# rasmusab/bayes.js

Hardware: AMD Instinct MI355X
Metric: posterior draws/sec (= param-updates/sec) (higher is better)
Workload: dtype f64

## Files before the change

bayes.js_amd/amwg_ctypes.py:

```python
import ctypes as C
import os

import numpy as np

HERE = os.path.dirname(os.path.abspath(__file__))
LIB_PATH = os.environ.get("AMWG_LIB") or os.path.join(HERE, "csrc", "libamwg.so")
MODEL_ID = {"normal": 1, "beta_bern": 2, "hier_normal": 3, "pois_glm": 4}


class ParamDesc(C.Structure):
    _fields_ = [("type", C.c_int32), ("len", C.c_int32), ("top", C.c_int32), ("multidim", C.c_int32),
                ("lower", C.c_double), ("upper", C.c_double)]


class CompOpt(C.Structure):
    _fields_ = [("prop_log_scale", C.c_double), ("max_adaptation", C.c_double), ("initial_adaptation", C.c_double),
                ("target_accept_rate", C.c_double), ("batch_size", C.c_double), ("is_adapting", C.c_int32)]


class ModelDesc(C.Structure):
    _fields_ = [("model", C.c_int32), ("n_obs", C.c_int32), ("x", C.POINTER(C.c_double)), ("y", C.POINTER(C.c_double)),
                ("g", C.POINTER(C.c_int32)), ("G", C.c_int32), ("K", C.c_int32), ("hyper", C.c_double * 8)]


DEFAULT_HYPER = {"normal": [0, 100, 0, 100], "beta_bern": [2, 2], "hier_normal": [0, 100, 0, 100, 10], "pois_glm": [0, 10]}


class Options(C.Structure):
    _fields_ = [("chains", C.c_int64), ("seed", C.c_uint64), ("chain_offset", C.c_uint64), ("device", C.c_int32),
                ("lanes_per_chain", C.c_int32), ("block_threads", C.c_int32), ("steps_per_launch", C.c_int32),
                ("exact_division", C.c_int32), ("group_local", C.c_int32), ("full_evaluation", C.c_int32), ("test_bound_shift", C.c_int32), ("sufficient_statistics", C.c_int32)]


class UserModel(C.Structure):
    _fields_ = [("source", C.c_char_p), ("n_arrays", C.c_int32), ("arrays", C.POINTER(C.POINTER(C.c_double))),
                ("array_len", C.POINTER(C.c_int64)), ("array_type", C.POINTER(C.c_int32)), ("n_derived", C.c_int32), ("lds_bytes", C.c_int32), ("lds_bytes_one_lane", C.c_int32),
                ("parallel", C.c_int32), ("max_threads", C.c_int32), ("work_per_eval", C.c_double), ("work_one_lane", C.c_double),
                ("rows_n_obs", C.c_int32), ("rows_groups", C.c_int32), ("rows_sweep", C.c_int32)]


EXPORTS = ["amwg_kernel_name", "amwg_summation_order", "amwg_group_gather_draws", "amwg_group_comm_info", "amwg_comm_unique_id", "amwg_comm_create", "amwg_comm_info", "amwg_comm_gather_draws", "amwg_comm_moments", "amwg_comm_destroy", "amwg_code_cache_stats", "amwg_tuning", "amwg_group_moments", "amwg_group_diagnostics", "amwg_group_quantiles", "amwg_last_sample_quantiles", "amwg_fp64_peak", "amwg_set_state", "amwg_last_sample_diagnostics", "amwg_create_user", "amwg_compile_user", "amwg_num_recorded", "amwg_create", "amwg_burn", "amwg_burn_async", "amwg_sample", "amwg_sample_async", "amwg_fetch_draws", "amwg_fetch_draws_slices", "amwg_sample_device", "amwg_set_adapting", "amwg_get_state", "amwg_info", "amwg_chain_diag", "amwg_last_sample_moments", "amwg_sync", "amwg_num_components", "amwg_num_chains", "amwg_launch_info", "amwg_destroy", "amwg_last_error", "amwg_version", "amwg_exp", "amwg_log", "amwg_uniform"]
SELFTEST_EXPORTS = ["amwg_prefault_selftest", "amwg_math1", "amwg_math2", "amwg_hypot3", "amwg_log1p", "amwg_expm1", "amwg_two_valued_sum_check", "amwg_pow", "amwg_ld_host", "amwg_ld_device", "amwg_device_eval"]

_lib = None


def lib():
    global _lib
    if _lib is None:
        if not os.path.exists(LIB_PATH):
            raise RuntimeError("libamwg.so is missing: run `python -c 'import __graft_entry__ as g; g.build()'`")
        L = C.CDLL(LIB_PATH)
        vp, i32, i64, u64, dbl = C.c_void_p, C.c_int32, C.c_int64, C.c_uint64, C.c_double
        pd, pi32, pi64, pu64 = C.POINTER(dbl), C.POINTER(i32), C.POINTER(i64), C.POINTER(u64)
        L.amwg_create.argtypes = [C.POINTER(ModelDesc), C.POINTER(ParamDesc), i32, pd, C.POINTER(CompOpt),
                                  C.POINTER(Options), C.POINTER(vp)]
        L.amwg_burn.argtypes = [vp, i64]
        L.amwg_burn_async.argtypes = [vp, i64]
        L.amwg_sample_async.argtypes = [vp, i64, i64]
        L.amwg_fetch_draws.argtypes = [vp, pd, C.c_size_t]
        L.amwg_fetch_draws_slices.argtypes = [vp, C.c_int32, C.POINTER(C.c_int32), C.POINTER(C.c_int32), C.POINTER(C.POINTER(C.c_double)), C.POINTER(C.c_size_t)]
        L.amwg_sample.argtypes = [vp, i64, i64, pd, C.c_size_t]
        L.amwg_sample_device.argtypes = [vp, i64, i64, vp, C.c_size_t]
        L.amwg_set_adapting.argtypes = [vp, i32]
        L.amwg_get_state.argtypes = [vp, pd, C.c_size_t]
        L.amwg_info.argtypes = [vp, pd, pi32, pi32, pi32, pi64, pi64]
        L.amwg_chain_diag.argtypes = [vp, pu64, pd, pi32]
        L.amwg_last_sample_moments.argtypes = [vp, pd, pd]
        L.amwg_sync.argtypes = [vp]
        L.amwg_num_components.argtypes = [vp]
        L.amwg_num_chains.argtypes = [vp]
        L.amwg_num_chains.restype = i64
        L.amwg_launch_info.argtypes = [vp, pi32, pi32, pi32, pi32, pi32, pd]
        L.amwg_kernel_name.argtypes = [vp]
        L.amwg_summation_order.argtypes = [vp]
        L.amwg_kernel_name.restype = C.c_char_p
        L.amwg_destroy.argtypes = [vp]
        L.amwg_last_error.restype = C.c_char_p
        L.amwg_version.restype = C.c_char_p
        L.amwg_exp.restype = dbl
        L.amwg_exp.argtypes = [dbl]
        L.amwg_log.restype = dbl
        L.amwg_log.argtypes = [dbl]
        L.amwg_uniform.restype = dbl
        L.amwg_uniform.argtypes = [u64, u64, u64]
        L.amwg_compile_user.argtypes = [C.c_char_p, i32, i32, C.c_char_p, C.POINTER(C.c_size_t)]
        L.amwg_code_cache_stats.argtypes = [pi64, pi64, C.c_char_p, C.c_size_t]
        L.amwg_create_user.argtypes = [C.POINTER(UserModel), C.POINTER(ParamDesc), i32, pd, C.POINTER(CompOpt),
                                       C.POINTER(Options), C.POINTER(vp)]
        L.amwg_num_recorded.argtypes = [vp]
        L.amwg_set_state.argtypes = [vp, pd, C.c_size_t]
        L.amwg_fp64_peak.argtypes = [i32, pd]
        L.amwg_last_sample_quantiles.argtypes = [vp, pd, i32, pd]
        L.amwg_last_sample_diagnostics.argtypes = [vp, pd, pd]
        pvp = C.POINTER(vp)
        L.amwg_group_moments.argtypes = [pvp, i32, pd, pd]
        L.amwg_group_diagnostics.argtypes = [pvp, i32, pd, pd]
        L.amwg_group_quantiles.argtypes = [pvp, i32, pd, i32, pd]
        L.amwg_group_gather_draws.argtypes = [pvp, i32, i32, vp, pd, C.c_size_t, pi64]
        L.amwg_group_comm_info.argtypes = [pvp, i32, pi32, pi32, i32]
        L.amwg_comm_unique_id.argtypes = [C.c_char_p, C.c_size_t]
        L.amwg_comm_create.argtypes = [C.c_char_p, C.c_size_t, i32, i32, i32, pvp]
        L.amwg_comm_info.argtypes = [vp, pi32, pi32, pi32]
        L.amwg_comm_gather_draws.argtypes = [vp, vp, i32, vp, C.c_size_t, pi64]
        L.amwg_comm_moments.argtypes = [vp, vp, pd, pd]
        L.amwg_comm_destroy.argtypes = [vp]
        _lib = L
    return _lib


_selftest = None


def selftest_lib():
    global _selftest
    if _selftest is None:
        path = os.path.join(os.path.dirname(LIB_PATH), "libamwg_selftest.so")
        if not os.path.exists(path):
            raise RuntimeError("libamwg_selftest.so is missing: run `python -c 'import __graft_entry__ as g; g.build()'`")
        L = C.CDLL(path)
        i32, i64, dbl = C.c_int32, C.c_int64, C.c_double
        pd = C.POINTER(dbl)
        L.amwg_last_error.restype = C.c_char_p
        L.amwg_device_eval.argtypes = [i32, i32, i64, pd, pd, pd, pd]
        L.amwg_two_valued_sum_check.argtypes = [i32, pd, i32, i64, pd, pd, pd, pd, pd]
        L.amwg_pow.restype = dbl
        L.amwg_pow.argtypes = [dbl, dbl]
        L.amwg_math1.restype = dbl
        L.amwg_math1.argtypes = [i32, dbl]
        L.amwg_math2.restype = dbl
        L.amwg_math2.argtypes = [i32, dbl, dbl]
        L.amwg_hypot3.restype = dbl
        L.amwg_hypot3.argtypes = [dbl, dbl, dbl]
        for f in ("amwg_log1p", "amwg_expm1"):
            getattr(L, f).restype = dbl
            getattr(L, f).argtypes = [dbl]
        L.amwg_ld_host.restype = dbl
        L.amwg_ld_host.argtypes = [i32, dbl, dbl, dbl, dbl]
        L.amwg_ld_device.argtypes = [i32, i64, pd, pd]
        L.amwg_prefault_selftest.argtypes = [C.c_void_p, C.c_size_t, i32, i32]
        _selftest = L
    return _selftest


class AmwgError(RuntimeError):
    pass


def _check(rc):
    if rc != 0:
        raise AmwgError("amwg error %d: %s" % (rc, lib().amwg_last_error().decode()))


def _dp(a):
    return a.ctypes.data_as(C.POINTER(C.c_double))


class Sampler:

    def __init__(self, spec, chains, seed, chain_offset=0, device=0, lanes_per_chain=0, block_threads=0,
                 steps_per_launch=0, exact_division=0, group_local=0, full_evaluation=0, test_bound_shift=0, sufficient_statistics=0):
        L = lib()
        keep = []
        user = spec.get("user")
        if user is None:
            d = spec["data"]
            md = ModelDesc()
            md.model = MODEL_ID[spec["model"]]
            md.n_obs = spec["n_obs"]
            x = np.ascontiguousarray(d["x"], dtype=np.float64)
            keep.append(x)
            md.x = _dp(x)
            if "y" in d:
                y = np.ascontiguousarray(d["y"], dtype=np.float64)
                keep.append(y)
                md.y = _dp(y)
            if "g" in d:
                g = np.ascontiguousarray(d["g"], dtype=np.int32)
                keep.append(g)
                md.g = g.ctypes.data_as(C.POINTER(C.c_int32))
            md.G = int(spec.get("G", 0))
            md.K = int(spec.get("K", 0))
            for i, v in enumerate(spec.get("hyper") or DEFAULT_HYPER[spec["model"]]):
                md.hyper[i] = float(v)
        else:
            um = UserModel()
            src = user["source"].encode() if isinstance(user["source"], str) else user["source"]
            keep.append(src)
            um.source = src
            arrs = [np.ascontiguousarray(a, dtype=np.float64) for a in user["arrays"]]
            keep.append(arrs)
            um.n_arrays = len(arrs)
            ptrs = (C.POINTER(C.c_double) * max(1, len(arrs)))(*[_dp(a) for a in arrs])
            lens = (C.c_int64 * max(1, len(arrs)))(*[a.size for a in arrs])
            types = (C.c_int32 * max(1, len(arrs)))(*[int(t) for t in user.get("array_types", [0] * len(arrs))])
            keep += [ptrs, lens, types]
            um.arrays, um.array_len, um.array_type = ptrs, lens, types
            um.n_derived, um.lds_bytes = int(user.get("n_derived", 0)), int(user.get("lds_bytes", 0))
            um.lds_bytes_one_lane = int(user.get("lds_bytes_one_lane", 0))
            um.parallel, um.max_threads = int(user.get("parallel", 0)), int(user.get("max_threads", 0))
            um.work_per_eval = float(user.get("work_per_eval", 0.0))
            um.work_one_lane = float(user.get("work_one_lane", 0.0))
            um.rows_n_obs, um.rows_groups, um.rows_sweep = int(user.get("rows_n_obs", 0)), int(user.get("rows_groups", 0)), int(user.get("rows_sweep", 0))
        n = len(spec["params"])
        pa = (ParamDesc * n)()
        TYPE = {"real": 0, "int": 1, "binary": 2}
        for i, p in enumerate(spec["params"]):
            pa[i].type = TYPE[p["type"]]
# ... 242 lines not shown
```

bayes.js_amd/csrc/amwg_models.h:

```cpp
#pragma once
#include "amwg_div.h"
#include "amwg_ld.h"
#include "amwg_pass.h"
#include "amwg_twoval.h"
#include "amwg_types.h"
#include "amwg_window.h"

namespace amwg {

__device__ __forceinline__ double norm_const_sd(double v, double m, double c_sd, double den, double y_hi, double y_lo, int den_ok) {
  const double t = v - m;
  const double tt = t * t;
  const double q = (den_ok && wide_range(tt)) ? div_by_invariant(tt, den, Reciprocal{y_hi, y_lo}) : tt / den;
  return c_sd - q;
}

struct NormCache {
  double sd, c, den;
  Reciprocal y;
  bool den_ok;
};
__device__ __forceinline__ NormCache norm_cache_init() { return NormCache{__builtin_nan(""), 0.0, 0.0, Reciprocal{0.0, 0.0}, false}; }
AMWG_HD NormCache norm_cache_make(double sd, double neg_half_log_2pi) {
  NormCache k;
  k.sd = sd;
  k.c = norm_c(neg_half_log_2pi, sd);
  k.den = norm_den(sd);
  k.y = make_reciprocal(k.den);
  k.den_ok = mid_range(k.den);
  return k;
}
struct NormCacheA { double c, den; };
AMWG_HD_OUTLINE NormCacheA norm_cache_cold_a(double sd, double neg_half_log_2pi) { return NormCacheA{norm_c(neg_half_log_2pi, sd), norm_den(sd)}; }
AMWG_HD_OUTLINE Reciprocal norm_cache_cold_b(double den) { return make_reciprocal(den); }
template <bool COLD = false>
__device__ __forceinline__ void norm_cache_update(NormCache &k, double sd, double neg_half_log_2pi) {
  if (sd != k.sd) {
    if constexpr (COLD) {
      const NormCacheA a = norm_cache_cold_a(sd, neg_half_log_2pi);
      k.sd = sd; k.c = a.c; k.den = a.den;
      k.y = norm_cache_cold_b(a.den);
      k.den_ok = mid_range(a.den);
    } else {
      k = norm_cache_make(sd, neg_half_log_2pi);
    }
  }
}



struct NormalModel {
  static constexpr bool kSplitPrior = false;
  static constexpr bool kUser = false, kHasFast = true, kOneLanePass = false;
  static constexpr int kDerived = 0;
  static constexpr bool kHasBinary = false;
  static constexpr int kMaxThreads = 1024;
  static constexpr int kUnroll = 8;
  struct Pass { double mu, c, den; Reciprocal y; bool fast; const double *x; };
  static constexpr size_t kOneLaneTileLimit = 96 * 1024;
  __host__ __device__ static size_t one_lane_tile_bytes(int n_obs) { return (size_t)n_obs * 8 <= kOneLaneTileLimit ? (size_t)n_obs * 8 : 0; }
  __host__ __device__ static size_t lds_bytes(int n_obs, int, int lanes) { return lanes == 1 ? 0 : (size_t)n_obs * 8; }
  static constexpr bool kDynamicLds = true;
  __host__ __device__ static size_t lds_bytes_of(const DataRef &d, int lanes, int) { return lanes == 1 ? (d.pad > 0 ? one_lane_tile_bytes(d.n_obs) : 0) : (size_t)d.n_obs * 8; }
  __device__ static void stage(unsigned char *smem, const DataRef &d, int tid, int nt, int lanes) {
    if (lanes == 1 && lds_bytes_of(d, 1, nt) == 0) return;
    double *dst = reinterpret_cast<double *>(smem);
    for (int i = tid; i < d.n_obs; i += nt) dst[i] = d.x[i];
  }
  template <class C>
  __device__ __forceinline__ static double prior(const StateView &, const ModelConsts &mc, const DataRef &, C &kc) {
    double lp = 0;
    lp += norm_const_sd(kc.mu, mc.m0, mc.c0, mc.den0, mc.y0_hi, mc.y0_lo, mc.den0_ok);
    const double sigma = kc.sigma;
    lp += (sigma < mc.ua || sigma > mc.ub) ? -kInf : mc.lunif;
    return lp;
  }
  static constexpr bool kTracksState = true;
  struct Cache { NormCache n; double mu, sigma; bool loaded; };
  __device__ __forceinline__ static Cache cache_init() { return Cache{norm_cache_init(), 0.0, 0.0, false}; }
  __device__ __forceinline__ static void on_set(Cache &k, int comp, double v, int, const DataRef &) { k.mu = comp == 0 ? v : k.mu; k.sigma = comp == 0 ? k.sigma : v; }
  static constexpr bool kMirrorCheck = true;
  template <int GL>
  __device__ __forceinline__ static bool mirror_ok(const Cache &k, const StateView &S, const DataRef &, int) {
    return !k.loaded || (f64_bits(k.mu) == f64_bits(S(0)) && f64_bits(k.sigma) == f64_bits(S(1)));
  }
  template <int GL>
  __device__ __forceinline__ static void load(Cache &k, const StateView &S, const ModelConsts &, const DataRef &, const unsigned char *, int) {
    if (!k.loaded) { k.mu = S(0); k.sigma = S(1); k.loaded = true; }
  }
  template <int GL>
  __device__ __forceinline__ static Pass begin(const StateView &, const ModelConsts &mc, const DataRef &d,
                                               const unsigned char *smem, Cache &kc) {
    Pass ps;
    NormCache &k = kc.n;
    ps.mu = kc.mu;
    norm_cache_update(k, kc.sigma, mc.neg_half_log_2pi);
    ps.c = k.c;
    ps.den = k.den;
    ps.y = k.y;
    ps.fast = !mc.exact_division && mc.data_mid_range && k.den_ok &&
              (ps.mu == 0 || mid_range(__builtin_fabs(ps.mu)));
    ps.x = GL == 1 ? d.x : reinterpret_cast<const double *>(smem);
    return ps;
  }
  template <bool FAST>
  __device__ __forceinline__ static double term(const Pass &ps, int i) {
    const double t = ps.x[i] - ps.mu;
    const double tt = t * t;
    return ps.c - (FAST ? div_by_invariant(tt, ps.den, ps.y) : tt / ps.den);
  }
  template <int G>
  __device__ inline __attribute__((noinline)) static double pass_slow_impl(const double *x, double mu, double c, double den, int n_obs, int sub, double acc) {
    for (int i = sub; i < n_obs; i += G) { const double t = x[i] - mu; acc += c - (t * t) / den; }
    return acc;
  }
  template <int G>
  __device__ __forceinline__ static double pass_slow(const Pass &ps, int n_obs, int sub, double acc) { return pass_slow_impl<G>(ps.x, ps.mu, ps.c, ps.den, n_obs, sub, acc); }
  static constexpr bool kStagedFast = true;
  template <int G, int U = 8>
  __device__ __forceinline__ static double pass_fast(const Pass &ps, int n_obs, int sub, double acc) {
    if constexpr (G == 1) return norm_pass_uniform<8>(ps.x, ps.mu, ps.c, ps.den, ps.y, n_obs, acc);
    else return norm_pass_staged<G, U, false>(ps.x, nullptr, StateView{nullptr}, ps.mu, ps.c, ps.den, ps.y, n_obs, sub, acc);
  }
  static constexpr bool kCertified = true;
  static constexpr int kCertifiedLanes = 1;
  struct Approx { double value, eps; };
  template <int G, int BT>
  __device__ __forceinline__ static Approx log_post_approx(Cache &kc, const StateView &S, const ModelConsts &mc, const DataRef &d, const unsigned char *smem, int sub) {
    static_assert(G == 1, "the certified pass of the Normal family is the one-lane one");
    load<G>(kc, S, mc, d, smem, sub);
    norm_cache_update(kc.n, kc.sigma, mc.neg_half_log_2pi);
    const double P = prior(S, mc, d, kc);
    double S2;
    if (mc.sufficient) {
      const double dm = (mc.suff_xbar_hi - kc.mu) + mc.suff_xbar_lo;
      S2 = __builtin_fma((double)d.n_obs, dm * dm, mc.suff_ss);
    } else
    if constexpr (BT <= 512) S2 = norm_sq_pass_wave<(BT <= 256 ? kWaveBlock : 8)>(lds_bytes_of(d, 1, 0) ? reinterpret_cast<const double *>(smem) : d.x, kc.mu, d.n_obs, wave_scratch_of(d));
    else S2 = norm_sq_pass_uniform<8>(d.x, kc.mu, d.n_obs);
    const double n = (double)d.n_obs;
    const double Q = S2 * kc.n.y.hi, nc = n * kc.n.c;
    const double mag = __builtin_fabs(P) + __builtin_fabs(nc) + 2.0 * Q;
    return Approx{(P + nc) - Q, (2.0 * n + 64.0) * 0x1p-53 * mag * 1.25};
  }
};

struct BetaBernModel {
  static constexpr bool kSplitPrior = false;
  static constexpr bool kUser = false, kHasFast = false, kOneLanePass = true;
  static constexpr int kDerived = 0;
  static constexpr bool kHasBinary = false;
  static constexpr int kMaxThreads = 1024;
  static constexpr int kUnroll = 8;
  struct Pass { double l1, l0; const uint8_t *x; const uint32_t *bits; bool has_invalid, fast_forward; BitData B; };
  __host__ __device__ static size_t words(int n_obs) { return (size_t)n_obs / 32 + 2; }
  static constexpr size_t kFfLdsLimit = 120 * 1024;
  __host__ __device__ static size_t lds_bytes(int n_obs, int, int lanes) {
    if (lanes == 1) { const size_t b = 6 * words(n_obs) * 4; return b <= kFfLdsLimit ? ((b + 15) & ~(size_t)15) : 0; }
    return ((size_t)n_obs + 15) & ~(size_t)15;
  }
  __device__ static void stage(unsigned char *smem, const DataRef &d, int tid, int nt, int lanes) {
    if (lanes == 1) {
      if (lds_bytes(d.n_obs, 0, 1) == 0) return;
      uint32_t *dst = reinterpret_cast<uint32_t *>(smem);
      const uint32_t *src = static_cast<const uint32_t *>(d.arr[0]);
      for (int k = tid; k < (int)(6 * words(d.n_obs)); k += nt) dst[k] = src[k];
      return;
    }
    for (int i = tid; i < d.n_obs; i += nt) smem[i] = d.xb[i];
  }
  template <class C>
  __device__ __forceinline__ static double prior(const StateView &S, const ModelConsts &mc, const DataRef &, C &) {
    const double th = S(0);
    double lp = 0;
    if (th > 1 || th < 0) lp += -kInf;
    else if (mc.ba == 1 && mc.bb == 1) lp += 0.0;
    else lp += (mc.ba - 1) * log_v8(th) + (mc.bb - 1) * log_v8(1 - th) - mc.lbeta_ab;
    return lp;
  }
  struct Cache {};
  __device__ __forceinline__ static Cache cache_init() { return Cache{}; }
  template <int GL>
  __device__ __forceinline__ static Pass begin(const StateView &S, const ModelConsts &mc, const DataRef &d,
                                               const unsigned char *smem, Cache &) {
    Pass ps;
    const double th = S(0);
    ps.l1 = log_v8(th);
    ps.l0 = log_v8(1 - th);
    ps.x = smem;
    ps.bits = d.xw;
    ps.has_invalid = mc.has_invalid != 0;
    ps.fast_forward = !mc.exact_division;
    {
      const size_t W = words(d.n_obs);
      const uint32_t *base = lds_bytes(d.n_obs, 0, 1) ? reinterpret_cast<const uint32_t *>(smem) : static_cast<const uint32_t *>(d.arr[0]);
      ps.B.w = base; ps.B.pre = base + W; ps.B.om1 = base + 2 * W; ps.B.po1 = base + 3 * W; ps.B.om0 = base + 4 * W; ps.B.po0 = base + 5 * W;
      ps.B.n = d.n_obs;
    }
    return ps;
  }
  template <bool FAST>
  __device__ __forceinline__ static double term(const Pass &ps, int i) { return ps.x[i] ? ps.l1 : ps.l0; }

#define AMWG_A0 "v_add_f64 %[acc], %[acc], %[l0]\n"
#define AMWG_A1 "v_add_f64 %[acc], %[acc], %[l1]\n"
#define AMWG_N0 AMWG_A0 AMWG_A0 AMWG_A0 AMWG_A0
#define AMWG_N1 AMWG_A1 AMWG_A0 AMWG_A0 AMWG_A0
#define AMWG_N2 AMWG_A0 AMWG_A1 AMWG_A0 AMWG_A0
#define AMWG_N3 AMWG_A1 AMWG_A1 AMWG_A0 AMWG_A0
#define AMWG_N4 AMWG_A0 AMWG_A0 AMWG_A1 AMWG_A0
#define AMWG_N5 AMWG_A1 AMWG_A0 AMWG_A1 AMWG_A0
#define AMWG_N6 AMWG_A0 AMWG_A1 AMWG_A1 AMWG_A0
#define AMWG_N7 AMWG_A1 AMWG_A1 AMWG_A1 AMWG_A0
#define AMWG_N8 AMWG_A0 AMWG_A0 AMWG_A0 AMWG_A1
#define AMWG_N9 AMWG_A1 AMWG_A0 AMWG_A0 AMWG_A1
#define AMWG_N10 AMWG_A0 AMWG_A1 AMWG_A0 AMWG_A1
#define AMWG_N11 AMWG_A1 AMWG_A1 AMWG_A0 AMWG_A1
#define AMWG_N12 AMWG_A0 AMWG_A0 AMWG_A1 AMWG_A1
#define AMWG_N13 AMWG_A1 AMWG_A0 AMWG_A1 AMWG_A1
#define AMWG_N14 AMWG_A0 AMWG_A1 AMWG_A1 AMWG_A1
#define AMWG_N15 AMWG_A1 AMWG_A1 AMWG_A1 AMWG_A1
// ... 805 lines not shown
```

bayes.js_amd/csrc/amwg_pass.h:

```cpp
#pragma once
#include "amwg_div.h"
#include "amwg_types.h"

namespace amwg {

#if defined(__HIP_DEVICE_COMPILE__)
#define AMWG_STAGE_FENCE() __builtin_amdgcn_sched_barrier(0)
#else
#define AMWG_STAGE_FENCE() ((void)0)
#endif

template <int U>
struct NormBlock { double v[U]; };

#if defined(__HIP_DEVICE_COMPILE__)
#define AMWG_WAIT_LDS_LE(n) __builtin_amdgcn_s_waitcnt(0xC07F | ((n) << 8))
#else
#define AMWG_WAIT_LDS_LE(n) ((void)0)
#endif

template <int U, bool ADD_PREV>
AMWG_HD void norm_block_stages(NormBlock<U> &b, const double (&m)[U], NormBlock<U> &q, const NormBlock<U> &prev, double &acc,
                                                  double c, double den, Reciprocal y) {
  int a = 0;
// ... 184 lines not shown
    compute(sb, StagedFirst{});
    int ch = 1;
    for (; ch + 1 < n_chunks; ch += 2) {
      AMWG_WAIT_LDS_LE(0); AMWG_STAGE_FENCE();
      load_chunk(ch + 1, sb);
      AMWG_STAGE_FENCE();
      compute(sa, StagedLater{});
      AMWG_WAIT_LDS_LE(0); AMWG_STAGE_FENCE();
      load_chunk(ch + 2, sa);
      AMWG_STAGE_FENCE();
      compute(sb, StagedLater{});
    }
    if (ch < n_chunks) {
      AMWG_WAIT_LDS_LE(0); AMWG_STAGE_FENCE();
      compute(sa, StagedLater{});
    }
#pragma unroll
    for (int u = 0; u < U; ++u) acc = acc + qb.v[u];
    k = n_chunks * CH;
  }
  for (; k < n_obs; ++k) {
    const double t = x_global[k] - mean;
    acc += c - div_by_invariant(t * t, den, y);
  }
  return acc;
}

template <int U>
AMWG_HD double norm_sq_pass_uniform(const double *x_global, double mean, int n_obs) {
  constexpr int CH = 2 * U;
  double acc[U];
#pragma unroll
  for (int u = 0; u < U; ++u) acc[u] = 0.0;
  const int n_chunks = n_obs / CH;
  int k = 0;
  if (n_chunks > 0) {
    amwg_uniform_f64_ptr px = (amwg_uniform_f64_ptr)(uintptr_t)x_global;
    NormBlock<CH> sa, sb;
    auto load_chunk = [&](int ch, NormBlock<CH> &dst) {
      ch = ch < n_chunks ? ch : n_chunks - 1;
#pragma unroll
      for (int u = 0; u < CH; ++u) dst.v[u] = px[ch * CH + u];
    };
    auto compute = [&](const NormBlock<CH> &src) {
#pragma unroll
      for (int u = 0; u < U; ++u) { const double t = src.v[u] - mean; acc[u] = __builtin_fma(t, t, acc[u]); }
      AMWG_STAGE_FENCE();
#pragma unroll
      for (int u = 0; u < U; ++u) { const double t = src.v[U + u] - mean; acc[u] = __builtin_fma(t, t, acc[u]); }
      AMWG_STAGE_FENCE();
    };
    load_chunk(0, sb);
    AMWG_WAIT_LDS_LE(0); AMWG_STAGE_FENCE();
    load_chunk(1, sa);
    AMWG_STAGE_FENCE();
    compute(sb);
    int ch = 1;
    for (; ch + 1 < n_chunks; ch += 2) {
      AMWG_WAIT_LDS_LE(0); AMWG_STAGE_FENCE();
      load_chunk(ch + 1, sb);
      AMWG_STAGE_FENCE();
      compute(sa);
      AMWG_WAIT_LDS_LE(0); AMWG_STAGE_FENCE();
      load_chunk(ch + 2, sa);
      AMWG_STAGE_FENCE();
      compute(sb);
    }
    if (ch < n_chunks) {
      AMWG_WAIT_LDS_LE(0); AMWG_STAGE_FENCE();
      compute(sa);
    }
    k = n_chunks * CH;
  }
  for (; k < n_obs; ++k) {
    const double t = x_global[k] - mean;
    acc[0] = __builtin_fma(t, t, acc[0]);
  }
  double s = 0.0;
#pragma unroll
  for (int u = 0; u < U; ++u) s += acc[u];
  return s;
}

#if defined(__HIPCC__) || defined(__HIPCC_RTC__)
#ifndef AMWG_WAVE_BLOCK
#define AMWG_WAVE_BLOCK 16
#endif
constexpr int kWaveBlock = AMWG_WAVE_BLOCK;
template <int N> struct PassBlock { static constexpr int value = N; };
typedef int amwg_v16i __attribute__((ext_vector_type(16)));
__device__ __forceinline__ double *wave_scratch_of(const DataRef &d) {
#if defined(__HIP_DEVICE_COMPILE__)
  if (!d.wave_scratch) return nullptr;
  const uint32_t wave = (uint32_t)__builtin_amdgcn_readfirstlane((int)(blockIdx.x * (blockDim.x >> 6) + (threadIdx.x >> 6)));
  return d.wave_scratch + (size_t)wave * 64;
#else
  (void)d; return nullptr;
#endif
}
template <int B>
__device__ __forceinline__ double norm_sq_pass_wave(const double *x, double mu, int n_obs, double *scr = nullptr) {
#if defined(__HIP_DEVICE_COMPILE__)
  const int lane = (int)(threadIdx.x & 63u);
  double a[64];
#pragma unroll
  for (int c = 0; c < 64; ++c) a[c] = 0.0;
  const int mu_lo = (int)(uint32_t)f64_bits(mu), mu_hi = (int)(uint32_t)(f64_bits(mu) >> 32);
  auto mean_of = [&](int c) { return bits_f64(((uint64_t)(uint32_t)__builtin_amdgcn_readlane(mu_hi, c) << 32) | (uint64_t)(uint32_t)__builtin_amdgcn_readlane(mu_lo, c)); };
  bool smem_done = false;
#if !defined(AMWG_X_NO_SMEM_MEANS)
  if (scr != nullptr) {
    scr[lane] = mu;
    asm volatile("s_waitcnt vmcnt(0)\n\ts_dcache_inv\n\ts_waitcnt lgkmcnt(0)" ::: "memory");
    auto fetch = [&](int g) { amwg_v16i r; asm volatile("s_load_dwordx16 %0, %1, %2" : "=&s"(r) : "s"(scr), "s"(g * 8)); return r; };
    auto landed = [&](amwg_v16i &r) { asm volatile("s_waitcnt lgkmcnt(0)" : "+s"(r)); };
    auto mean_in = [&](const amwg_v16i &r, int j) { return bits_f64(((uint64_t)(uint32_t)r[2 * j + 1] << 32) | (uint64_t)(uint32_t)r[2 * j]); };
    auto block_s = [&](auto tag, int at) {
      constexpr int BB = decltype(tag)::value;
      double xv[BB];
      amwg_v16i cur = fetch(0);
#pragma unroll
      for (int b = 0; b < BB; ++b) xv[b] = x[at + b * 64 + lane];
#pragma unroll
      for (int g = 0; g < 64; g += 8) {
        landed(cur);
        amwg_v16i nxt = cur;
        if (g + 8 < 64) nxt = fetch(g + 8);
#pragma unroll
        for (int b = 0; b < BB; ++b) {
#pragma unroll
          for (int j = 0; j < 8; ++j) { const double t = xv[b] - mean_in(cur, j); a[g + j] = __builtin_fma(t, t, a[g + j]); }
        }
        cur = nxt;
      }
    };
    int base = 0;
    for (; base + 64 * B <= n_obs; base += 64 * B) block_s(PassBlock<B>{}, base);
    if constexpr (B >= 32) { if (base + 64 * 16 <= n_obs) { block_s(PassBlock<16>{}, base); base += 64 * 16; } }
    if constexpr (B >= 16) { if (base + 64 * 8 <= n_obs) { block_s(PassBlock<8>{}, base); base += 64 * 8; } }
    if constexpr (B >= 8) { if (base + 64 * 4 <= n_obs) { block_s(PassBlock<4>{}, base); base += 64 * 4; } }
    if constexpr (B >= 4) { if (base + 64 * 2 <= n_obs) { block_s(PassBlock<2>{}, base); base += 64 * 2; } }
    for (; base + 64 <= n_obs; base += 64) block_s(PassBlock<1>{}, base);
    if (base < n_obs) {
      const int i = base + lane;
      const bool has = i < n_obs;
      const double xv = x[has ? i : base];
      amwg_v16i cur = fetch(0);
#pragma unroll
      for (int g = 0; g < 64; g += 8) {
        landed(cur);
        amwg_v16i nxt = cur;
        if (g + 8 < 64) nxt = fetch(g + 8);
#pragma unroll
        for (int j = 0; j < 8; ++j) { const double t = has ? xv - mean_in(cur, j) : 0.0; a[g + j] = __builtin_fma(t, t, a[g + j]); }
        cur = nxt;
      }
    }
    smem_done = true;
  }
#endif
  if (!smem_done) {
  auto block = [&](auto tag, int at) {
    constexpr int BB = decltype(tag)::value;
    double xv[BB];
#pragma unroll
    for (int b = 0; b < BB; ++b) xv[b] = x[at + b * 64 + lane];
#pragma unroll
    for (int g = 0; g < 64; g += 8) {
      double m[8];
#pragma unroll
      for (int j = 0; j < 8; ++j) m[j] = mean_of(g + j);
#pragma unroll
      for (int b = 0; b < BB; ++b) {
#pragma unroll
        for (int j = 0; j < 8; ++j) { const double t = xv[b] - m[j]; a[g + j] = __builtin_fma(t, t, a[g + j]); }
      }
    }
  };
  int base = 0;
  for (; base + 64 * B <= n_obs; base += 64 * B) block(PassBlock<B>{}, base);
  if constexpr (B >= 32) { if (base + 64 * 16 <= n_obs) { block(PassBlock<16>{}, base); base += 64 * 16; } }
  if constexpr (B >= 16) { if (base + 64 * 8 <= n_obs) { block(PassBlock<8>{}, base); base += 64 * 8; } }
  if constexpr (B >= 8) { if (base + 64 * 4 <= n_obs) { block(PassBlock<4>{}, base); base += 64 * 4; } }
  if constexpr (B >= 4) { if (base + 64 * 2 <= n_obs) { block(PassBlock<2>{}, base); base += 64 * 2; } }
  if constexpr (B >= 2) { if (base + 64 <= n_obs) { block(PassBlock<1>{}, base); base += 64; } }
  for (; base + 64 <= n_obs; base += 64) block(PassBlock<1>{}, base);
  if (base < n_obs) {
    const int i = base + lane;
    const bool has = i < n_obs;
    const double xv = x[has ? i : base];
#pragma unroll
    for (int g = 0; g < 64; g += 8) {
      double m[8];
#pragma unroll
      for (int j = 0; j < 8; ++j) m[j] = mean_of(g + j);
#pragma unroll
      for (int j = 0; j < 8; ++j) { const double t = has ? xv - m[j] : 0.0; a[g + j] = __builtin_fma(t, t, a[g + j]); }
    }
  }
  }
  auto swap_add = [&](double A, double Bv, int off) {
    const uint32_t al = (uint32_t)f64_bits(A), ah = (uint32_t)(f64_bits(A) >> 32), bl = (uint32_t)f64_bits(Bv), bh = (uint32_t)(f64_bits(Bv) >> 32);
    if (off == 32) {
      const auto l = __builtin_amdgcn_permlane32_swap(al, bl, false, false), h = __builtin_amdgcn_permlane32_swap(ah, bh, false, false);
      return bits_f64(((uint64_t)h[0] << 32) | (uint64_t)l[0]) + bits_f64(((uint64_t)h[1] << 32) | (uint64_t)l[1]);
    } else {
      const auto l = __builtin_amdgcn_permlane16_swap(al, bl, false, false), h = __builtin_amdgcn_permlane16_swap(ah, bh, false, false);
      return bits_f64(((uint64_t)h[0] << 32) | (uint64_t)l[0]) + bits_f64(((uint64_t)h[1] << 32) | (uint64_t)l[1]);
    }
  };
#pragma unroll
  for (int j = 0; j < 32; ++j) a[j] = swap_add(a[j], a[j + 32], 32);
#pragma unroll
  for (int j = 0; j < 16; ++j) a[j] = swap_add(a[j], a[j + 16], 16);
  {
    const bool up = (lane & 8) != 0;
#pragma unroll
    for (int j = 0; j < 8; ++j) { const double send = up ? a[j] : a[j + 8], keep = up ? a[j + 8] : a[j]; a[j] = keep + xor_partner<8, true>(send); }
  }
  {
    const bool up = (lane & 4) != 0;
#pragma unroll
    for (int j = 0; j < 4; ++j) { const double send = up ? a[j] : a[j + 4], keep = up ? a[j + 4] : a[j]; a[j] = keep + xor_partner<4, true>(send); }
  }
  {
    const bool up = (lane & 2) != 0;
#pragma unroll
    for (int j = 0; j < 2; ++j) { const double send = up ? a[j] : a[j + 2], keep = up ? a[j + 2] : a[j]; a[j] = keep + xor_partner<2>(send); }
  }
  {
    const bool up = (lane & 1) != 0;
    const double send = up ? a[0] : a[1], keep = up ? a[1] : a[0];
    a[0] = keep + xor_partner<1>(send);
  }
  return a[0];
#else
  (void)x; (void)mu; (void)n_obs;
  return 0.0;
#endif
}
#endif

}
```

bayes.js_amd/csrc/amwg_selftest.hip:

```cpp
#include "../../include/amwg_selftest.h"
#include "amwg_eval.h"
#include "amwg_host.h"
#include "amwg_kernel.h"
#include "amwg_models.h"

using namespace amwg;
__global__ void two_valued_check_kernel(const uint32_t *tab, int N, int64_t m, const double *acc0, const double *l1, const double *l0,
                                        double *out_ff, double *out_seq) {
  const int64_t j = (int64_t)blockIdx.x * blockDim.x + threadIdx.x;
  if (j >= m) return;
  const size_t W = BetaBernModel::words(N);
  BitData B{tab, tab + W, tab + 2 * W, tab + 3 * W, tab + 4 * W, tab + 5 * W, N};
  out_ff[j] = two_valued_sum(acc0[j], l1[j], l0[j], B);
  double acc = acc0[j];
  for (int i = 0; i < N; ++i) acc = acc + (((tab[i >> 5] >> (i & 31)) & 1u) ? l1[j] : l0[j]);
  out_seq[j] = acc;
}

extern "C" {
double amwg_pow(double x, double y) { return pow_v8(x, y); }
double amwg_log1p(double x) { return log1p_v8(x); }
double amwg_expm1(double x) { return expm1_v8(x); }
double amwg_math1(int32_t fn, double x) { return math1_by_id(fn, x); }
double amwg_math2(int32_t fn, double x, double y) {
  switch (fn) {
    case 0: return atan2_v8(x, y);
    case 1: return hypot2_v8(x, y);
    case 2: return js_mod(x, y);
    case 3: return (double)js_toint32(x);
  }
  return __builtin_nan("");
}
double amwg_hypot3(double x, double y, double z) { return hypot3_v8(x, y, z); }
double amwg_ld_host(int32_t id, double x, double a, double b, double c) { return ld_by_id(id, x, a, b, c); }

int amwg_prefault_selftest(char *buf, size_t bytes, int32_t n_chunks, int32_t threads) {
  if (!buf || n_chunks < 1 || threads < 0 || threads > 16) return amwg_fail(AMWG_EINVAL, "amwg_prefault_selftest: bad argument");
  Prefaulter pf((size_t)n_chunks);
  const size_t per = bytes / (size_t)n_chunks;
  for (int32_t j = 0; j < n_chunks; ++j) pf.add(buf + (size_t)j * per, j == n_chunks - 1 ? bytes - (size_t)j * per : per, (size_t)j);
  pf.start(threads);
  for (int32_t j = 0; j < n_chunks; ++j) pf.wait_chunk((size_t)j);
  return AMWG_OK;
}

int amwg_two_valued_sum_check(int32_t device, const double *x, int32_t n, int64_t m, const double *acc0, const double *l1, const double *l0,
                              double *out_fast_forward, double *out_term_by_term) {
  if (!x || !acc0 || !l1 || !l0 || !out_fast_forward || !out_term_by_term || n < 0 || m < 0) return amwg_fail(AMWG_EINVAL, "amwg_two_valued_sum_check: bad argument");
  TRYB(use_device(device));
  std::vector<uint8_t> xb((size_t)n);
  for (int i = 0; i < n; ++i) xb[i] = x[i] == 1 ? 1 : 0;
  const std::vector<uint32_t> tab = two_valued_tables(xb.data(), n);
  DevBuf dtab, d[5];
  HIP_TRY(dtab.alloc(tab.size() * 4));
  HIP_TRY(hipMemcpy(dtab.p, tab.data(), tab.size() * 4, hipMemcpyHostToDevice));
  const double *src[3] = {acc0, l1, l0};
  for (int k = 0; k < 5; ++k) {
    HIP_TRY(d[k].alloc((size_t)m * 8));
    if (k < 3 && m) HIP_TRY(hipMemcpy(d[k].p, src[k], (size_t)m * 8, hipMemcpyHostToDevice));
  }
  if (m) hipLaunchKernelGGL(two_valued_check_kernel, dim3((unsigned)((m + 63) / 64)), dim3(64), 0, 0, dtab.as<uint32_t>(), n, m,
                            d[0].as<double>(), d[1].as<double>(), d[2].as<double>(), d[3].as<double>(), d[4].as<double>());
  HIP_TRY(hipGetLastError());
  HIP_TRY(hipMemcpy(out_fast_forward, d[3].p, (size_t)m * 8, hipMemcpyDeviceToHost));
  HIP_TRY(hipMemcpy(out_term_by_term, d[4].p, (size_t)m * 8, hipMemcpyDeviceToHost));
  return AMWG_OK;
}

int amwg_ld_device(int32_t device, int64_t n, const double *records, double *out) {
  if (!records || !out || n < 0) return amwg_fail(AMWG_EINVAL, "amwg_ld_device: bad argument");
  TRYB(use_device(device));
  DevBuf dr, dout;
  HIP_TRY(dr.alloc((size_t)n * 40));
  HIP_TRY(dout.alloc((size_t)n * 8));
  HIP_TRY(hipMemcpy(dr.p, records, (size_t)n * 40, hipMemcpyHostToDevice));
  if (n) hipLaunchKernelGGL(amwg_ld_eval_kernel, dim3((unsigned)((n + 255) / 256)), dim3(256), 0, 0, n, dr.as<double>(), dout.as<double>());
  HIP_TRY(hipGetLastError());
  HIP_TRY(hipMemcpy(out, dout.p, (size_t)n * 8, hipMemcpyDeviceToHost));
  return AMWG_OK;
}

int amwg_device_eval(int32_t device, int32_t op, int64_t n, const double *a, const double *b, const double *c, double *out) {
  if (!a || !out || n < 0) return amwg_fail(AMWG_EINVAL, "amwg_device_eval: bad argument");
  TRYB(use_device(device));
  DevBuf da, db, dc, dout;
  const size_t bytes = (size_t)n * 8;
  HIP_TRY(da.alloc(bytes));
  HIP_TRY(dout.alloc(bytes));
  HIP_TRY(hipMemcpy(da.p, a, bytes, hipMemcpyHostToDevice));
  if (b) { HIP_TRY(db.alloc(bytes)); HIP_TRY(hipMemcpy(db.p, b, bytes, hipMemcpyHostToDevice)); }
  if (c) { HIP_TRY(dc.alloc(bytes)); HIP_TRY(hipMemcpy(dc.p, c, bytes, hipMemcpyHostToDevice)); }
  if (n) hipLaunchKernelGGL(amwg_eval_kernel, dim3((unsigned)((n + 255) / 256)), dim3(256), 0, 0, op, n, da.as<double>(), db.as<double>(), dc.as<double>(), dout.as<double>());
  HIP_TRY(hipGetLastError());
  HIP_TRY(hipMemcpy(out, dout.p, bytes, hipMemcpyDeviceToHost));
  return AMWG_OK;
}

}
```

include/amwg_selftest.h:

```cpp
#ifndef AMWG_SELFTEST_H
#define AMWG_SELFTEST_H
#include "amwg.h"
#ifdef __cplusplus
extern "C" {
#endif

int amwg_device_eval(int32_t device, int32_t op, int64_t n, const double *a, const double *b, const double *c, double *out);
double amwg_pow(double x, double y);
double amwg_log1p(double x);
double amwg_expm1(double x);
double amwg_math1(int32_t fn, double x);
double amwg_math2(int32_t fn, double x, double y);
double amwg_hypot3(double x, double y, double z);
double amwg_ld_host(int32_t id, double x, double a, double b, double c);
int amwg_ld_device(int32_t device, int64_t n, const double *records, double *out);
int amwg_two_valued_sum_check(int32_t device, const double *x, int32_t n, int64_t m, const double *acc0, const double *l1, const double *l0,
                              double *out_fast_forward, double *out_term_by_term);

int amwg_prefault_selftest(char *buf, size_t bytes, int32_t n_chunks, int32_t threads);

#if defined(AMWG_AUDIT) || defined(AMWG_X_PHASES)
int amwg_audit_fetch(amwg_sampler *s, double *per_chain, uint64_t *hist, int32_t reset);
#endif

#ifdef __cplusplus
}
#endif
#endif
```

Measured before the change: 1.421 billion.

## Double-buffer observation loads and pipeline scalar mean fetches in wave sum-of-squares pass

Restructures the per-wave squared-deviation pass for the normal model so the next block of observations is loaded while the current block is computed, with scalar-memory loads of the 64 chain means issued one group ahead. It also skips republishing the means to scratch (and the cache invalidate) when the wave's means match the last published ones, and uses an LDS address-space pointer when the data tile lives in shared memory. The tail rounds are loaded in one go rather than block by block. The cost is more VGPR pressure from two register buffers and more complex inline-asm ordering, and a selftest entry point is added to check the new path.

```diff
diff --git a/bayes.js_amd/amwg_ctypes.py b/bayes.js_amd/amwg_ctypes.py
--- a/bayes.js_amd/amwg_ctypes.py
+++ b/bayes.js_amd/amwg_ctypes.py
@@ -40,7 +40,7 @@
 
 
 EXPORTS = ["amwg_kernel_name", "amwg_summation_order", "amwg_group_gather_draws", "amwg_group_comm_info", "amwg_comm_unique_id", "amwg_comm_create", "amwg_comm_info", "amwg_comm_gather_draws", "amwg_comm_moments", "amwg_comm_destroy", "amwg_code_cache_stats", "amwg_tuning", "amwg_group_moments", "amwg_group_diagnostics", "amwg_group_quantiles", "amwg_last_sample_quantiles", "amwg_fp64_peak", "amwg_set_state", "amwg_last_sample_diagnostics", "amwg_create_user", "amwg_compile_user", "amwg_num_recorded", "amwg_create", "amwg_burn", "amwg_burn_async", "amwg_sample", "amwg_sample_async", "amwg_fetch_draws", "amwg_fetch_draws_slices", "amwg_sample_device", "amwg_set_adapting", "amwg_get_state", "amwg_info", "amwg_chain_diag", "amwg_last_sample_moments", "amwg_sync", "amwg_num_components", "amwg_num_chains", "amwg_launch_info", "amwg_destroy", "amwg_last_error", "amwg_version", "amwg_exp", "amwg_log", "amwg_uniform"]
-SELFTEST_EXPORTS = ["amwg_prefault_selftest", "amwg_math1", "amwg_math2", "amwg_hypot3", "amwg_log1p", "amwg_expm1", "amwg_two_valued_sum_check", "amwg_pow", "amwg_ld_host", "amwg_ld_device", "amwg_device_eval"]
+SELFTEST_EXPORTS = ["amwg_prefault_selftest", "amwg_math1", "amwg_math2", "amwg_hypot3", "amwg_log1p", "amwg_expm1", "amwg_two_valued_sum_check", "amwg_norm_sq_pass_check", "amwg_pow", "amwg_ld_host", "amwg_ld_device", "amwg_device_eval"]
 
 _lib = None
 
@@ -124,6 +124,7 @@
         L.amwg_last_error.restype = C.c_char_p
         L.amwg_device_eval.argtypes = [i32, i32, i64, pd, pd, pd, pd]
         L.amwg_two_valued_sum_check.argtypes = [i32, pd, i32, i64, pd, pd, pd, pd, pd]
+        L.amwg_norm_sq_pass_check.argtypes = [i32, pd, i32, pd, i32, i32, i32, i32, pd, C.POINTER(i32)]
         L.amwg_pow.restype = dbl
         L.amwg_pow.argtypes = [dbl, dbl]
         L.amwg_math1.restype = dbl
diff --git a/bayes.js_amd/csrc/amwg_models.h b/bayes.js_amd/csrc/amwg_models.h
--- a/bayes.js_amd/csrc/amwg_models.h
+++ b/bayes.js_amd/csrc/amwg_models.h
@@ -76,8 +76,8 @@
     return lp;
   }
   static constexpr bool kTracksState = true;
-  struct Cache { NormCache n; double mu, sigma; bool loaded; };
-  __device__ __forceinline__ static Cache cache_init() { return Cache{norm_cache_init(), 0.0, 0.0, false}; }
+  struct Cache { NormCache n; double mu, sigma; bool loaded; WaveMeans published; };
+  __device__ __forceinline__ static Cache cache_init() { return Cache{norm_cache_init(), 0.0, 0.0, false, wave_means_init()}; }
   __device__ __forceinline__ static void on_set(Cache &k, int comp, double v, int, const DataRef &) { k.mu = comp == 0 ? v : k.mu; k.sigma = comp == 0 ? k.sigma : v; }
   static constexpr bool kMirrorCheck = true;
   template <int GL>
@@ -136,7 +136,7 @@
       const double dm = (mc.suff_xbar_hi - kc.mu) + mc.suff_xbar_lo;
       S2 = __builtin_fma((double)d.n_obs, dm * dm, mc.suff_ss);
     } else
-    if constexpr (BT <= 512) S2 = norm_sq_pass_wave<(BT <= 256 ? kWaveBlock : 8)>(lds_bytes_of(d, 1, 0) ? reinterpret_cast<const double *>(smem) : d.x, kc.mu, d.n_obs, wave_scratch_of(d));
+    if constexpr (BT <= 512) S2 = norm_sq_pass_wave<(BT <= 256 ? kWaveBlock : 8), (BT <= 256)>(lds_bytes_of(d, 1, 0) ? reinterpret_cast<const double *>(smem) : d.x, kc.mu, d.n_obs, wave_scratch_of(d), &kc.published);
     else S2 = norm_sq_pass_uniform<8>(d.x, kc.mu, d.n_obs);
     const double n = (double)d.n_obs;
     const double Q = S2 * kc.n.y.hi, nc = n * kc.n.c;
diff --git a/bayes.js_amd/csrc/amwg_pass.h b/bayes.js_amd/csrc/amwg_pass.h
--- a/bayes.js_amd/csrc/amwg_pass.h
+++ b/bayes.js_amd/csrc/amwg_pass.h
@@ -290,6 +290,8 @@
   return s;
 }
 
+struct WaveMeans { double mu; bool valid; int publishes; };
+AMWG_HD WaveMeans wave_means_init() { return WaveMeans{0.0, false, 0}; }
 #if defined(__HIPCC__) || defined(__HIPCC_RTC__)
 #ifndef AMWG_WAVE_BLOCK
 #define AMWG_WAVE_BLOCK 16
@@ -306,107 +308,135 @@
   (void)d; return nullptr;
 #endif
 }
-template <int B>
-__device__ __forceinline__ double norm_sq_pass_wave(const double *x, double mu, int n_obs, double *scr = nullptr) {
-#if defined(__HIP_DEVICE_COMPILE__)
+#if defined(__HIP_DEVICE_COMPILE__)
+typedef const double __attribute__((address_space(3))) *amwg_lds_f64_ptr;
+#endif
+template <int N> struct PassAt { static constexpr int value = N; };
+template <bool V> struct PassFlag { static constexpr bool value = V; };
+
+template <int B, bool SM, bool DB, class XP>
+__device__ __forceinline__ double norm_sq_pass_wave_in(XP x, double mu, int n_obs, double *scr, WaveMeans *pub) {
+#if defined(__HIP_DEVICE_COMPILE__)
+  static_assert(B >= 2 && B <= 32 && (B & (B - 1)) == 0, "rounds per block: a power of two");
   const int lane = (int)(threadIdx.x & 63u);
   double a[64];
-#pragma unroll
-  for (int c = 0; c < 64; ++c) a[c] = 0.0;
+  double xa[B], xb[DB ? B : 1];
   const int mu_lo = (int)(uint32_t)f64_bits(mu), mu_hi = (int)(uint32_t)(f64_bits(mu) >> 32);
   auto mean_of = [&](int c) { return bits_f64(((uint64_t)(uint32_t)__builtin_amdgcn_readlane(mu_hi, c) << 32) | (uint64_t)(uint32_t)__builtin_amdgcn_readlane(mu_lo, c)); };
-  bool smem_done = false;
-#if !defined(AMWG_X_NO_SMEM_MEANS)
-  if (scr != nullptr) {
-    scr[lane] = mu;
-    asm volatile("s_waitcnt vmcnt(0)\n\ts_dcache_inv\n\ts_waitcnt lgkmcnt(0)" ::: "memory");
-    auto fetch = [&](int g) { amwg_v16i r; asm volatile("s_load_dwordx16 %0, %1, %2" : "=&s"(r) : "s"(scr), "s"(g * 8)); return r; };
-    auto landed = [&](amwg_v16i &r) { asm volatile("s_waitcnt lgkmcnt(0)" : "+s"(r)); };
-    auto mean_in = [&](const amwg_v16i &r, int j) { return bits_f64(((uint64_t)(uint32_t)r[2 * j + 1] << 32) | (uint64_t)(uint32_t)r[2 * j]); };
-    auto block_s = [&](auto tag, int at) {
-      constexpr int BB = decltype(tag)::value;
-      double xv[BB];
-      amwg_v16i cur = fetch(0);
-#pragma unroll
-      for (int b = 0; b < BB; ++b) xv[b] = x[at + b * 64 + lane];
-#pragma unroll
-      for (int g = 0; g < 64; g += 8) {
-        landed(cur);
-        amwg_v16i nxt = cur;
-        if (g + 8 < 64) nxt = fetch(g + 8);
-#pragma unroll
-        for (int b = 0; b < BB; ++b) {
-#pragma unroll
-          for (int j = 0; j < 8; ++j) { const double t = xv[b] - mean_in(cur, j); a[g + j] = __builtin_fma(t, t, a[g + j]); }
-        }
-        cur = nxt;
+  auto mean_in = [&](const amwg_v16i &r, int j) { return bits_f64(((uint64_t)(uint32_t)r[2 * j + 1] << 32) | (uint64_t)(uint32_t)r[2 * j]); };
+  auto fetch = [&](amwg_v16i &r, int g) { asm volatile("s_load_dwordx16 %0, %1, %2" : "=&s"(r) : "s"(scr), "s"(g * 8) : "memory"); };
+  auto wait_fetch = [&](amwg_v16i &have, amwg_v16i &next, int g) {
+    asm volatile("s_waitcnt lgkmcnt(0)\n\ts_load_dwordx16 %0, %2, %3" : "=&s"(next), "+s"(have) : "s"(scr), "s"(g * 8) : "memory");
+  };
+  auto wait_for = [&](amwg_v16i &have) { asm volatile("s_waitcnt lgkmcnt(0)" : "+s"(have) : : "memory"); };
+  amwg_v16i ma, mb;
+
+  const int n_whole = n_obs / (64 * B);
+  const int rest_at = n_whole * 64 * B;
+  const int rest_rounds = (n_obs - rest_at) >> 6;
+  const bool rest_masked = (n_obs & 63) != 0;
+  const bool has_last = ((rest_at + (rest_rounds << 6)) + lane) < n_obs;
+  auto load_block = [&](double (&xv)[B], int at) {
+#pragma unroll
+    for (int b = 0; b < B; ++b) xv[b] = x[at + b * 64 + lane];
+  };
+  auto load_rest = [&](double (&xv)[B]) {
+    int at = rest_at;
+#pragma unroll
+    for (int L = B / 2; L >= 1; L >>= 1) {
+      if (rest_rounds & L) {
+#pragma unroll
+        for (int b = 0; b < L; ++b) xv[B - 2 * L + b] = x[at + b * 64 + lane];
+        at += 64 * L;
       }
-    };
-    int base = 0;
-    for (; base + 64 * B <= n_obs; base += 64 * B) block_s(PassBlock<B>{}, base);
-    if constexpr (B >= 32) { if (base + 64 * 16 <= n_obs) { block_s(PassBlock<16>{}, base); base += 64 * 16; } }
-    if constexpr (B >= 16) { if (base + 64 * 8 <= n_obs) { block_s(PassBlock<8>{}, base); base += 64 * 8; } }
-    if constexpr (B >= 8) { if (base + 64 * 4 <= n_obs) { block_s(PassBlock<4>{}, base); base += 64 * 4; } }
-    if constexpr (B >= 4) { if (base + 64 * 2 <= n_obs) { block_s(PassBlock<2>{}, base); base += 64 * 2; } }
-    for (; base + 64 <= n_obs; base += 64) block_s(PassBlock<1>{}, base);
-    if (base < n_obs) {
-      const int i = base + lane;
-      const bool has = i < n_obs;
-      const double xv = x[has ? i : base];
-      amwg_v16i cur = fetch(0);
-#pragma unroll
-      for (int g = 0; g < 64; g += 8) {
-        landed(cur);
-        amwg_v16i nxt = cur;
-        if (g + 8 < 64) nxt = fetch(g + 8);
-#pragma unroll
-        for (int j = 0; j < 8; ++j) { const double t = has ? xv - mean_in(cur, j) : 0.0; a[g + j] = __builtin_fma(t, t, a[g + j]); }
-        cur = nxt;
+    }
+    if (rest_masked) xv[B - 1] = x[has_last ? at + lane : at];
+  };
+  auto arith = [&](auto bb, auto first, auto masked, const double (&xv)[B], int g, const amwg_v16i &ms) {
+    constexpr int BB = decltype(bb)::value, FIRST = decltype(first)::value;
+    double m[8];
+#pragma unroll
+    for (int j = 0; j < 8; ++j) m[j] = SM ? mean_in(ms, j) : mean_of(g + j);
+#pragma unroll
+    for (int b = 0; b < BB; ++b) {
+#pragma unroll
+      for (int j = 0; j < 8; ++j) {
+        const double d = xv[FIRST + b] - m[j];
+        const double t = decltype(masked)::value ? (has_last ? d : 0.0) : d;
+        a[g + j] = __builtin_fma(t, t, a[g + j]);
       }
     }
-    smem_done = true;
-  }
-#endif
-  if (!smem_done) {
-  auto block = [&](auto tag, int at) {
-    constexpr int BB = decltype(tag)::value;
-    double xv[BB];
-#pragma unroll
-    for (int b = 0; b < BB; ++b) xv[b] = x[at + b * 64 + lane];
-#pragma unroll
-    for (int g = 0; g < 64; g += 8) {
-      double m[8];
-#pragma unroll
-      for (int j = 0; j < 8; ++j) m[j] = mean_of(g + j);
-#pragma unroll
-      for (int b = 0; b < BB; ++b) {
-#pragma unroll
-        for (int j = 0; j < 8; ++j) { const double t = xv[b] - m[j]; a[g + j] = __builtin_fma(t, t, a[g + j]); }
-      }
-    }
-  };
-  int base = 0;
-  for (; base + 64 * B <= n_obs; base += 64 * B) block(PassBlock<B>{}, base);
-  if constexpr (B >= 32) { if (base + 64 * 16 <= n_obs) { block(PassBlock<16>{}, base); base += 64 * 16; } }
-  if constexpr (B >= 16) { if (base + 64 * 8 <= n_obs) { block(PassBlock<8>{}, base); base += 64 * 8; } }
-  if constexpr (B >= 8) { if (base + 64 * 4 <= n_obs) { block(PassBlock<4>{}, base); base += 64 * 4; } }
-  if constexpr (B >= 4) { if (base + 64 * 2 <= n_obs) { block(PassBlock<2>{}, base); base += 64 * 2; } }
-  if constexpr (B >= 2) { if (base + 64 <= n_obs) { block(PassBlock<1>{}, base); base += 64; } }
-  for (; base + 64 <= n_obs; base += 64) block(PassBlock<1>{}, base);
-  if (base < n_obs) {
-    const int i = base + lane;
-    const bool has = i < n_obs;
-    const double xv = x[has ? i : base];
-#pragma unroll
-    for (int g = 0; g < 64; g += 8) {
-      double m[8];
-#pragma unroll
-      for (int j = 0; j < 8; ++j) m[j] = mean_of(g + j);
-#pragma unroll
-      for (int j = 0; j < 8; ++j) { const double t = has ? xv - m[j] : 0.0; a[g + j] = __builtin_fma(t, t, a[g + j]); }
-    }
-  }
-  }
+  };
+  auto done = [&](int g) {
+    asm volatile("" : "+v"(a[g]), "+v"(a[g + 1]), "+v"(a[g + 2]), "+v"(a[g + 3]), "+v"(a[g + 4]), "+v"(a[g + 5]), "+v"(a[g + 6]), "+v"(a[g + 7]));
+  };
+  auto block = [&](auto bb, auto first, auto masked, auto enter, auto leave, const double (&xv)[B], auto ahead) {
+    if constexpr (SM && !decltype(enter)::value) fetch(ma, 0);
+#pragma unroll
+    for (int g = 0; g < 64; g += 16) {
+      if constexpr (SM) { if (g == 0) { wait_for(ma); AMWG_WAIT_LDS_LE(0); } else wait_fetch(ma, mb, g + 8); }
+      if (g == 0) { ahead(); if constexpr (SM) fetch(mb, 8); }
+      AMWG_STAGE_FENCE();
+      arith(bb, first, masked, xv, g, ma);
+      done(g);
+      AMWG_STAGE_FENCE();
+      if constexpr (SM) { if (g + 16 < 64 || decltype(leave)::value) wait_fetch(mb, ma, (g + 16) & 63); else wait_for(mb); }
+      AMWG_STAGE_FENCE();
+      arith(bb, first, masked, xv, g + 8, mb);
+      done(g + 8);
+      AMWG_STAGE_FENCE();
+    }
+  };
+  auto nothing = [] {};
+  constexpr PassFlag<true> yes{};
+  constexpr PassFlag<false> no{};
+  auto rest = [&](const double (&xv)[B]) {
+    if constexpr (B >= 32) { if (rest_rounds & 16) block(PassBlock<16>{}, PassAt<B - 32>{}, no, no, no, xv, nothing); }
+    if constexpr (B >= 16) { if (rest_rounds & 8) block(PassBlock<8>{}, PassAt<B - 16>{}, no, no, no, xv, nothing); }
+    if constexpr (B >= 8) { if (rest_rounds & 4) block(PassBlock<4>{}, PassAt<B - 8>{}, no, no, no, xv, nothing); }
+    if constexpr (B >= 4) { if (rest_rounds & 2) block(PassBlock<2>{}, PassAt<B - 4>{}, no, no, no, xv, nothing); }
+    if (rest_rounds & 1) block(PassBlock<1>{}, PassAt<B - 2>{}, no, no, no, xv, nothing);
+    if (rest_masked) block(PassBlock<1>{}, PassAt<B - 1>{}, yes, no, no, xv, nothing);
+  };
+
+  bool publish = false;
+  if constexpr (SM) {
+    const bool same = pub != nullptr && pub->valid && f64_bits(pub->mu) == f64_bits(mu);
+    publish = __builtin_amdgcn_ballot_w64(!same) != 0;
+    if (publish) scr[lane] = mu;
+  }
+  if (n_whole > 0) load_block(xa, 0); else load_rest(xa);
+#pragma unroll
+  for (int c = 0; c < 64; ++c) a[c] = 0.0;
+  AMWG_STAGE_FENCE();
+  if constexpr (SM) {
+    if (publish) {
+      asm volatile("s_waitcnt vmcnt(0)\n\ts_dcache_inv\n\ts_waitcnt lgkmcnt(0)" ::: "memory");
+      if (pub != nullptr) { pub->mu = mu; pub->valid = true; pub->publishes += 1; }
+    }
+  }
+  if constexpr (DB) {
+    int k = 0;
+#pragma nounroll
+    for (; k + 2 <= n_whole; k += 2) {
+      block(PassBlock<B>{}, PassAt<0>{}, no, no, yes, xa, [&] { load_block(xb, (k + 1) * 64 * B); });
+      block(PassBlock<B>{}, PassAt<0>{}, no, yes, no, xb, [&] { if (k + 2 < n_whole) load_block(xa, (k + 2) * 64 * B); else load_rest(xa); });
+    }
+    if (k < n_whole) {
+      block(PassBlock<B>{}, PassAt<0>{}, no, no, no, xa, [&] { load_rest(xb); });
+      rest(xb);
+    } else {
+      rest(xa);
+    }
+  } else {
+#pragma nounroll
+    for (int k = 0; k < n_whole; ++k) {
+      block(PassBlock<B>{}, PassAt<0>{}, no, no, no, xa, nothing);
+      if (k + 1 < n_whole) load_block(xa, (k + 1) * 64 * B); else load_rest(xa);
+    }
+    rest(xa);
+  }
+
   auto swap_add = [&](double A, double Bv, int off) {
     const uint32_t al = (uint32_t)f64_bits(A), ah = (uint32_t)(f64_bits(A) >> 32), bl = (uint32_t)f64_bits(Bv), bh = (uint32_t)(f64_bits(Bv) >> 32);
     if (off == 32) {
@@ -443,10 +473,28 @@
   }
   return a[0];
 #else
-  (void)x; (void)mu; (void)n_obs;
+  (void)x; (void)mu; (void)n_obs; (void)scr; (void)pub;
   return 0.0;
 #endif
 }
-#endif
-
-}
+
+template <int B, bool DB = true>
+__device__ __forceinline__ double norm_sq_pass_wave(const double *x, double mu, int n_obs, double *scr = nullptr, WaveMeans *pub = nullptr) {
+#if defined(__HIP_DEVICE_COMPILE__)
+  const bool in_lds = __builtin_amdgcn_is_shared((const void *)x);
+#if !defined(AMWG_X_NO_SMEM_MEANS)
+  if (scr != nullptr) {
+    if (in_lds) return norm_sq_pass_wave_in<B, true, DB>((amwg_lds_f64_ptr)x, mu, n_obs, scr, pub);
+    return norm_sq_pass_wave_in<B, true, DB>(x, mu, n_obs, scr, pub);
+  }
+#endif
+  if (in_lds) return norm_sq_pass_wave_in<B, false, DB>((amwg_lds_f64_ptr)x, mu, n_obs, nullptr, nullptr);
+  return norm_sq_pass_wave_in<B, false, DB>(x, mu, n_obs, nullptr, nullptr);
+#else
+  (void)x; (void)mu; (void)n_obs; (void)scr; (void)pub;
+  return 0.0;
+#endif
+}
+#endif
+
+}
diff --git a/bayes.js_amd/csrc/amwg_selftest.hip b/bayes.js_amd/csrc/amwg_selftest.hip
--- a/bayes.js_amd/csrc/amwg_selftest.hip
+++ b/bayes.js_amd/csrc/amwg_selftest.hip
@@ -15,6 +15,23 @@
   double acc = acc0[j];
   for (int i = 0; i < N; ++i) acc = acc + (((tab[i >> 5] >> (i & 31)) & 1u) ? l1[j] : l0[j]);
   out_seq[j] = acc;
+}
+
+template <int B>
+__global__ void norm_sq_pass_check_kernel(const double *x, int n, const double *means, int calls, int tile, double *scr, double *out, int32_t *published) {
+  extern __shared__ __attribute__((aligned(16))) unsigned char check_lds[];
+  const int lane = (int)(threadIdx.x & 63u);
+  double *staged = reinterpret_cast<double *>(check_lds);
+  if (tile) {
+    for (int i = lane; i < n; i += 64) staged[i] = x[i];
+    __syncthreads();
+  }
+  WaveMeans pub = wave_means_init();
+  for (int c = 0; c < calls; ++c) {
+    const int before = pub.publishes;
+    out[c * 64 + lane] = norm_sq_pass_wave<B>(tile ? staged : x, means[c * 64 + lane], n, scr, &pub);
+    if (lane == 0) published[c] = pub.publishes - before;
+  }
 }
 
 extern "C" {
@@ -67,6 +84,31 @@
   return AMWG_OK;
 }
 
+int amwg_norm_sq_pass_check(int32_t device, const double *x, int32_t n, const double *means, int32_t calls, int32_t tile_in_lds, int32_t use_scratch, int32_t block_rounds,
+                            double *out, int32_t *published) {
+  if (!x || !means || !out || !published || n < 1 || calls < 1 || (block_rounds != 8 && block_rounds != 16) || (tile_in_lds && (size_t)n * 8 > 60 * 1024))
+    return amwg_fail(AMWG_EINVAL, "amwg_norm_sq_pass_check: bad argument");
+  TRYB(use_device(device));
+  DevBuf dx, dm, dscr, dout, dpub;
+  HIP_TRY(dx.alloc((size_t)n * 8));
+  HIP_TRY(dm.alloc((size_t)calls * 64 * 8));
+  HIP_TRY(dscr.alloc(64 * 8));
+  HIP_TRY(dout.alloc((size_t)calls * 64 * 8));
+  HIP_TRY(dpub.alloc((size_t)calls * 4));
+  HIP_TRY(hipMemcpy(dx.p, x, (size_t)n * 8, hipMemcpyHostToDevice));
+  HIP_TRY(hipMemcpy(dm.p, means, (size_t)calls * 64 * 8, hipMemcpyHostToDevice));
+  HIP_TRY(hipMemset(dscr.p, 0xff, 64 * 8));
+  HIP_TRY(hipMemset(dpub.p, 0, (size_t)calls * 4));
+  const size_t lds = tile_in_lds ? (size_t)n * 8 : 0;
+  double *scr = use_scratch ? dscr.as<double>() : nullptr;
+  if (block_rounds == 16) hipLaunchKernelGGL(norm_sq_pass_check_kernel<16>, dim3(1), dim3(64), lds, 0, dx.as<double>(), n, dm.as<double>(), calls, tile_in_lds, scr, dout.as<double>(), dpub.as<int32_t>());
+  else hipLaunchKernelGGL(norm_sq_pass_check_kernel<8>, dim3(1), dim3(64), lds, 0, dx.as<double>(), n, dm.as<double>(), calls, tile_in_lds, scr, dout.as<double>(), dpub.as<int32_t>());
+  HIP_TRY(hipGetLastError());
+  HIP_TRY(hipMemcpy(out, dout.p, (size_t)calls * 64 * 8, hipMemcpyDeviceToHost));
+  HIP_TRY(hipMemcpy(published, dpub.p, (size_t)calls * 4, hipMemcpyDeviceToHost));
+  return AMWG_OK;
+}
+
 int amwg_ld_device(int32_t device, int64_t n, const double *records, double *out) {
   if (!records || !out || n < 0) return amwg_fail(AMWG_EINVAL, "amwg_ld_device: bad argument");
   TRYB(use_device(device));
diff --git a/include/amwg_selftest.h b/include/amwg_selftest.h
--- a/include/amwg_selftest.h
+++ b/include/amwg_selftest.h
@@ -17,6 +17,9 @@
 int amwg_two_valued_sum_check(int32_t device, const double *x, int32_t n, int64_t m, const double *acc0, const double *l1, const double *l0,
                               double *out_fast_forward, double *out_term_by_term);
 
+int amwg_norm_sq_pass_check(int32_t device, const double *x, int32_t n, const double *means, int32_t calls, int32_t tile_in_lds, int32_t use_scratch, int32_t block_rounds,
+                            double *out, int32_t *published);
+
 int amwg_prefault_selftest(char *buf, size_t bytes, int32_t n_chunks, int32_t threads);
 
 #if defined(AMWG_AUDIT) || defined(AMWG_X_PHASES)
```

Result: no change. 1.409 billion (-0.9%).
